# arthur-e/MOD16

Measured on AMD Instinct MI355X. Metric: pixels/sec, fused Penman-Monteith ET forward run (day+night), 43200x21600 global grid, higher is better.
Workload: dtype f64

## Files before the change

### mod16_amd/csrc/capi/internal.hpp

```cpp
#pragma once
#include <hip/hip_runtime.h>

#include <algorithm>
#include <cmath>
#include <cstdio>
#include <cstdlib>
#include <cstring>
#include <limits>
#include <mutex>
#include <new>
#include <string>
#include <thread>
#include <vector>

#include "../../../include/mod16_hip.h"
#include "own.hpp"
#include "../mod16_kernels.hpp"
#include "../mod16_stream.hpp"

using namespace mod16;

namespace {
constexpr int kDiagBlocks = 1024;
constexpr int kSlots = 12;
// ... 105 lines not shown
        used += align256(bytes);
        return p;
    }
};

static void derive_lut(const double* lut, double* h64) {
    const double nan = std::numeric_limits<double>::quiet_NaN();
    for (int c = 0; c < kLutCols; ++c) {
        double row[MOD16_LUT_ROWS];
        for (int k = 0; k < MOD16_LUT_ROWS; ++k) row[k] = nan;
        if (c < MOD16_N_CLASSES) {
            const double* p = lut + (size_t)c * MOD16_N_PARAMS;
            for (int k = 0; k < MOD16_N_PARAMS; ++k) row[k] = p[k];
            row[11] = 1.0 / (p[MOD16_TMIN_OPEN] - p[MOD16_TMIN_CLOSE]);
            row[12] = 1.0 / (p[MOD16_VPD_CLOSE] - p[MOD16_VPD_OPEN]);
            row[13] = (p[MOD16_RBL_MAX] - p[MOD16_RBL_MIN]) / (p[MOD16_VPD_CLOSE] - p[MOD16_VPD_OPEN]);
            row[14] = 1.0 / p[MOD16_BETA];
            const double thr = 273.15 + p[MOD16_TMIN_CLOSE];
            float tf = (float)thr;
            if ((double)tf < thr) tf = std::nextafterf(tf, std::numeric_limits<float>::infinity());
            row[15] = (double)tf;
        }
        for (int k = 0; k < MOD16_LUT_ROWS; ++k) h64[k * kLutCols + c] = row[k];
    }
}

template <typename T> static const T* ctx_lut(const mod16_ctx* ctx);
template <> const double* ctx_lut<double>(const mod16_ctx* ctx) { return ctx->lut64.as<double>(); }
template <> const float* ctx_lut<float>(const mod16_ctx* ctx) { return ctx->lut32.as<float>(); }


// ... 485 lines not shown
```

### mod16_amd/csrc/mod16_composite.hpp

```cpp
#pragma once
#include "mod16_kernels.hpp"

namespace mod16 {

constexpr int kCompArrays = 15;
constexpr int kCompHours = 14;
constexpr int kCompMaxDays = 4096;

template <typename T> struct CompArgs {
    const T* arr[kCompArrays];
    int64_t tstride[kCompArrays];
    int every[kCompArrays];
    uint32_t dense;
    const uint8_t* cls;
    const double* lut64;
    const double* tab;
    T* out_et;
    T* out_pet;
    uint16_t* cnt_et;
    uint16_t* cnt_pet;
    int64_t out_pitch, cnt_pitch, n;
    int days, period_days, min_valid, rescale;
    unsigned* status;
};
// ... 36 lines not shown
__device__ __forceinline__ ClassPar<double> comp_params(const double* l) {
    ClassPar<double> p;
    p.tmin_close = l[0 * kLutCols];
    p.tmin_open = l[1 * kLutCols];
    p.vpd_open = l[2 * kLutCols];
    p.vpd_close = l[3 * kLutCols];
    p.gl_sh = l[4 * kLutCols];
    p.gl_wv = l[5 * kLutCols];
    p.g_cut = l[6 * kLutCols];
    p.csl = l[7 * kLutCols];
    p.rbl_min = l[8 * kLutCols];
    p.rbl_max = l[9 * kLutCols];
    p.beta = l[10 * kLutCols];
    p.inv_dtmin = l[11 * kLutCols];
    p.inv_dvpd = l[12 * kLutCols];
    p.rbl_slope = l[13 * kLutCols];
    p.inv_beta = l[14 * kLutCols];
    return p;
}

__device__ __forceinline__ PixelIn<double> comp_pixel(const double (&v)[kCompArrays]) {
    return PixelIn<double>{v[0], v[1], v[2], v[3], v[4], v[5], v[6], v[7], v[8], v[9], v[10], v[11], v[12], v[13]};
}

template <bool PET>
__device__ __forceinline__ void comp_totals(const PixelOut<double>& o, double h, double& et, double& pet) {
#pragma clang fp contract(off)
    et = comp_daily((o.canopy_d + o.soil_d) + o.trans_d, (o.canopy_n + o.soil_n) + o.trans_n, h);
    pet = PET ? comp_daily(o.pet_d, o.pet_n, h) : 0.0;
}

// ... 156 lines not shown
```

### mod16_amd/csrc/mod16_ensemble.hpp

```cpp
#pragma once
#include "mod16_kernels.hpp"

namespace mod16 {

constexpr int kEnsChunk = 16;
constexpr int kEnsTable = MOD16_LUT_ROWS * kLutCols;
constexpr int64_t kEnsMaxMembers = 65536;
constexpr int kEnsOut = 5;

template <typename T> struct EnsArgs {
    const T* drv[14];
    const uint8_t* cls;
    const double* tables;
    const double* tab;
    T* out[kEnsOut];
    int64_t n;
    int members;
    unsigned* status;
    uint32_t dense_drv;
};

struct EnsPeriod {
    double vpd, logrh, fwet, omw, s, slhv, inv_rcorr, g_rr;
    double rf;
// ... 90 lines not shown

struct EnsMember {
    double vpd_open, inv_dvpd, rbl_min, drbl, inv_beta, gl_sh, g_cut, csl_mt, glsh_lai, glwv_lai;
    bool cond;
};
__device__ __forceinline__ EnsMember ens_member(const EnsPixel& px, const double* l) {
#pragma clang fp contract(off)
    EnsMember m;
    const double tmin_close = l[0 * kLutCols];
    m.vpd_open = l[2 * kLutCols];
    m.gl_sh = l[4 * kLutCols];
    const double gl_wv = l[5 * kLutCols];
    m.g_cut = l[6 * kLutCols];
    const double csl = l[7 * kLutCols];
    m.rbl_min = l[8 * kLutCols];
    const double rbl_max = l[9 * kLutCols];
    const double inv_dtmin = l[11 * kLutCols];
    m.inv_dvpd = l[12 * kLutCols];
    m.inv_beta = l[14 * kLutCols];
    m.cond = px.base_cond & (px.t_ann >= (273.15 + tmin_close));
    m.glsh_lai = m.gl_sh * px.lai;
    m.glwv_lai = gl_wv * px.lai;
    m.drbl = rbl_max - m.rbl_min;
    typedef FastMath<double> M;
    m.csl_mt = csl * M::nan_from(M::mul_unit(px.tm - tmin_close, inv_dtmin), px.tm);
    return m;
}

template <bool DAY>
__device__ __forceinline__ double ens_period_eval(const EnsPixel& px, const EnsPeriod& c, const EnsMember& m,
                                                  const double* tb) {
#pragma clang fp contract(off)
    typedef FastMath<double> M;
    const double tiny = 1e-7;
    const double vramp = M::mul_unit(c.vpd - m.vpd_open, m.inv_dvpd);
    double canopy, soil, trans;
    {
        const double g_e = m.glwv_lai * c.fwet;
// ... 437 lines not shown
```

### mod16_amd/csrc/mod16_kernels.hpp

```cpp
#pragma once
#include <stdint.h>
#include <type_traits>
#include "mod16_physics.hpp"

namespace mod16 {

constexpr int kBlock = 256;
constexpr int kLutCols = 16;
constexpr unsigned kStatusClassRange = 1u;
constexpr unsigned kStatusIncomplete = 2u;
constexpr int kSerialField = 3;
__device__ __forceinline__ double launch_marker(unsigned serial) { return (double)((serial & 0xffffu) + 1u); }

template <typename T> struct EtArgs {
    const T* drv[14];
    const T* par[11];
    const uint8_t* cls;
    const T* lut;
    const double* lut64;
    const double* tab;
    T* out[10];
    int64_t n;
    unsigned* status;
    uint32_t dense_drv;
// ... 126 lines not shown
                const C* l = lut + c;
                p.tmin_close = l[0 * kLutCols];
                p.tmin_open = l[1 * kLutCols];
                p.vpd_open = l[2 * kLutCols];
                p.vpd_close = l[3 * kLutCols];
                p.gl_sh = l[4 * kLutCols];
                p.gl_wv = l[5 * kLutCols];
                p.g_cut = l[6 * kLutCols];
                p.csl = l[7 * kLutCols];
                p.rbl_min = l[8 * kLutCols];
                p.rbl_max = l[9 * kLutCols];
                p.beta = l[10 * kLutCols];
                if (FAST) {
                    p.inv_dtmin = l[11 * kLutCols];
                    p.inv_dvpd = l[12 * kLutCols];
                    p.rbl_slope = l[13 * kLutCols];
                    p.inv_beta = l[14 * kLutCols];
                }
            } else {
                p.tmin_close = (C)par(0);
                p.tmin_open = (C)par(1);
                p.vpd_open = (C)par(2);
                p.vpd_close = (C)par(3);
                p.gl_sh = (C)par(4);
                p.gl_wv = (C)par(5);
                p.g_cut = (C)par(6);
                p.csl = (C)par(7);
                p.rbl_min = (C)par(8);
                p.rbl_max = (C)par(9);
                p.beta = (C)par(10);
                if (FAST) p.derive();
// ... 331 lines not shown
```

### mod16_amd/csrc/mod16_math.hpp

```cpp
#pragma once
#ifndef MOD16_EXPERIMENTS
#if defined(MOD16_TRIVIAL_BODY) || defined(MOD16_NO_GUARD) || defined(MOD16_EXPERIMENT_SEED_RCP) || \
    defined(MOD16_PRIO) || defined(MOD16_REPRO_V4) || defined(MOD16_NO_FUSED_FINAL) ||                \
    defined(MOD16_NO_REDO_LAUNCH) || defined(MOD16_KK_M) || defined(MOD16_NO_FMA_KK) ||               \
    defined(MOD16_DYN_RUN) || defined(MOD16_MIXED_NO_CANCEL) || defined(MOD16_MIXED_CANCEL) || defined(MOD16_F64_CAND)
#error "MOD16_* measurement switches need -DMOD16_EXPERIMENTS (they are not part of the product build)"
#endif
#endif
#include <hip/hip_runtime.h>

namespace mod16 {

__device__ __forceinline__ void ignore_signalling_nans() {
    asm volatile("s_setreg_imm32_b32 hwreg(HW_REG_MODE, 9, 1), 0\n\ts_nop 3" ::: "memory");
}

__device__ __forceinline__ double in_vgpr(double k) {
    asm("" : "+v"(k));
    return k;
}

template <typename T> struct ExactMath {
    static __device__ __forceinline__ T exp(T x);
    static __device__ __forceinline__ T pow(T x, T y);
};
template <> __device__ __forceinline__ double ExactMath<double>::exp(double x) { return ::exp(x); }
template <> __device__ __forceinline__ float ExactMath<float>::exp(float x) { return ::expf(x); }
template <> __device__ __forceinline__ double ExactMath<double>::pow(double x, double y) { return ::pow(x, y); }
template <> __device__ __forceinline__ float ExactMath<float>::pow(float x, float y) { return ::powf(x, y); }

template <typename T> struct FastMath;

template <> struct FastMath<double> {
// ... 54 lines not shown
#else
        return rcp(x);
#endif
    }

    static __device__ __forceinline__ T pow_m1p75(T x) {
        T y = __builtin_amdgcn_sqrt(__builtin_amdgcn_rsq(x));
        T y2 = y * y;
        T t = x * (y2 * y2);
        y = y * fma_kk(t, -0.25, 1.25);
        y2 = y * y;
        T y4 = y2 * y2;
        return (y4 * y2) * y;
    }

    static __device__ __forceinline__ T pow_m1p75_rcp(T x, T& rx) {
        T y = __builtin_amdgcn_sqrt(__builtin_amdgcn_rsq(x));
        T y2 = y * y;
        T t = x * (y2 * y2);
        y = y * fma_kk(t, -0.25, 1.25);
        y2 = y * y;
        T y4 = y2 * y2;
        rx = y4;
        return (y4 * y2) * y;
    }

    static constexpr int kTabRaw = 64 + 2 * 128;
    static constexpr int kTabDoubles = kTabRaw + 16;
    static constexpr double kRintShift = 6755399441055744.0;

    static __device__ __forceinline__ T exp_tab(T x, const T* tb) {
        T km = __builtin_fma(x, 92.33248261689366, kRintShift);
        T kf = km - kRintShift;
        T r = __builtin_fma(kf, -0x1.62e42fee00000p-7, x);
        r = __builtin_fma(kf, -0x1.a39ef35793c76p-39, r);
// ... 7 lines not shown
    }

    static __device__ __forceinline__ T exp_tab4(T x, const T* tb) {
        T km = __builtin_fma(x, 92.33248261689366, kRintShift);
        T kf = km - kRintShift;
        T r = __builtin_fma(kf, -0x1.62e42fee00000p-7, x);
        r = __builtin_fma(kf, -0x1.a39ef35793c76p-39, r);
        T p = fma_kk(r, 1.0 / 24.0, 1.0 / 6.0);
        p = __builtin_fma(p, r, 0.5);
        p = __builtin_fma(p, r, 1.0);
        p = __builtin_fma(p, r, 1.0);
        int ki = __double2loint(km);
        return __builtin_amdgcn_ldexp(tb[ki & 63] * p, ki >> 6);
    }

    static __device__ __forceinline__ T exp_tab4s(T x, const T* tb) {
        T km = __builtin_fma(x, 92.33248261689366, kRintShift);
        T kf = km - kRintShift;
        T r = __builtin_fma(kf, -0.010830424696249145, x);
        T p = fma_kk(r, 1.0 / 24.0, 1.0 / 6.0);
        p = __builtin_fma(p, r, 0.5);
        p = __builtin_fma(p, r, 1.0);
        p = __builtin_fma(p, r, 1.0);
        int ki = __double2loint(km);
        return __builtin_amdgcn_ldexp(tb[ki & 63] * p, ki >> 6);
    }

    static __device__ __forceinline__ T exp_tab5s(T x, const T* tb) {
        T km = __builtin_fma(x, 92.33248261689366, kRintShift);
        T kf = km - kRintShift;
        T r = __builtin_fma(kf, -0.010830424696249145, x);
        T p = fma_kk(r, 1.0 / 120.0, 1.0 / 24.0);
        p = __builtin_fma(p, r, 1.0 / 6.0);
        p = __builtin_fma(p, r, 0.5);
        p = __builtin_fma(p, r, 1.0);
        p = __builtin_fma(p, r, 1.0);
        int ki = __double2loint(km);
        return __builtin_amdgcn_ldexp(tb[ki & 63] * p, ki >> 6);
    }

    static __device__ __forceinline__ T exp_tab3(T x, const T* tb) {
        T km = __builtin_fma(x, 92.33248261689366, kRintShift);
        T kf = km - kRintShift;
        T r = __builtin_fma(kf, -0x1.62e42fee00000p-7, x);
        r = __builtin_fma(kf, -0x1.a39ef35793c76p-39, r);
        T p = fma_kk(r, 1.0 / 6.0, 0.5);
        p = __builtin_fma(p, r, 1.0);
// ... 16 lines not shown
    static __device__ __forceinline__ T log_tab(T x, const T* tb) {
        const unsigned hi = (unsigned)__double2hiint(x);
        const int e = (int)(hi >> 20) - 1023;
        const unsigned j = (hi >> 13) & 127u;
        const T m = __hiloint2double((int)((hi & 0x000fffffu) | 0x3ff00000u), __double2loint(x));
        typedef double d2 __attribute__((ext_vector_type(2)));
        const d2 ent = *reinterpret_cast<const d2*>(tb + 64 + 2 * j);
        T r = __builtin_fma(m, ent[0], -1.0);
        T l1p = log1p_poly(r);
        T ed = (T)e;
        T v = __builtin_fma(ed, 0x1.62e42fefa2000p-1, ent[1]);
        v = v + l1p;
        v = __builtin_fma(ed, 7.371002565167799e-13, v);
        return (x == 0.0) ? -__builtin_huge_val() : v;
    }
    static __device__ __forceinline__ T log_tab1(T x, const T* tb) {
        const unsigned hi = (unsigned)__double2hiint(x);
        const int e = (int)(hi >> 20) - 1023;
        const unsigned j = (hi >> 13) & 127u;
        const T m = __hiloint2double((int)((hi & 0x000fffffu) | 0x3ff00000u), __double2loint(x));
        typedef double d2 __attribute__((ext_vector_type(2)));
        const d2 ent = *reinterpret_cast<const d2*>(tb + 64 + 2 * j);
        T r = __builtin_fma(m, ent[0], -1.0);
        T v = __builtin_fma((T)e, 0.6931471805599453, ent[1]) + log1p_poly(r);
        return (x == 0.0) ? -__builtin_huge_val() : v;
    }
    static __host__ __device__ __forceinline__ T log1p_poly(T r) {
#if defined(__HIP_DEVICE_COMPILE__)
        T p = fma_kk(r, 0.2, -0.25);
#else
        T p = __builtin_fma(r, 0.2, -0.25);
#endif
        p = __builtin_fma(p, r, 1.0 / 3.0);
        p = __builtin_fma(p, r, -0.5);
        return __builtin_fma(r * r, p, r);
    }

    static __device__ __forceinline__ T pow01_tab(T x, T y, const T* tb) {
        T yc = vmin_k(y, 1e300);
        T t = vmax_k(yc * log_tab(x, tb), -746.0);
        return exp_tab4(t, tb);
    }
    static __device__ __forceinline__ T pow01_tab1(T x, T y, const T* tb) {
        T yc = vmin_k(y, 1e300);
        T t = vmax_k(yc * log_tab1(x, tb), -746.0);
        return exp_tab4s(t, tb);
    }
};

}
```

### mod16_amd/csrc/mod16_methods.hpp

```cpp
#pragma once
#include "mod16_kernels.hpp"

namespace mod16 {

constexpr int kMethodMaxIn = 13;

template <typename T> struct MethodArgs {
    const T* in[kMethodMaxIn];
    const T* par[11];
    T* out[2];
    int64_t n;
    uint32_t dense_in, present_in, dense_par;
    int method;
    T alpha;
    T tiny;
};

template <typename T>
__global__ void __launch_bounds__(kBlock) method_kernel(const MethodArgs<T> a) {
    const int64_t step = (int64_t)gridDim.x * kBlock;
    for (int64_t i = (int64_t)blockIdx.x * kBlock + threadIdx.x; i < a.n; i += step) {
        auto has = [&](int k) { return (a.present_in >> k) & 1u; };
        auto in = [&](int k) { return ((a.dense_in >> k) & 1u) ? a.in[k][i] : a.in[k][0]; };
        auto par = [&](int k) { return ((a.dense_par >> k) & 1u) ? a.par[k][i] : a.par[k][0]; };
// ... 743 lines not shown
                      d(12), d(13), a.fpar_pct[i], a.lai_x10[i]};
        unsigned c = a.cls[i];
        if (c >= 13u) {
            atomicOr(a.status, kStatusClassRange);
            c = 13u;
        }
        const C* l = lut + c;
        ClassPar<C> p;
        p.tmin_close = l[0 * kLutCols]; p.tmin_open = l[1 * kLutCols];
        p.vpd_open = l[2 * kLutCols]; p.vpd_close = l[3 * kLutCols];
        p.gl_sh = l[4 * kLutCols]; p.gl_wv = l[5 * kLutCols];
        p.g_cut = l[6 * kLutCols]; p.csl = l[7 * kLutCols];
        p.rbl_min = l[8 * kLutCols]; p.rbl_max = l[9 * kLutCols];
        p.beta = l[10 * kLutCols];
        p.inv_dtmin = l[11 * kLutCols]; p.inv_dvpd = l[12 * kLutCols];
        p.rbl_slope = l[13 * kLutCols]; p.inv_beta = l[14 * kLutCols];
        PixelOut<C> o;
        if constexpr (FAST) {
            double dav_d, dav_n;
            const PixelIn<double> x = raw_to_pixel_fast(r, tab, dav_d, dav_n);
            o = et_pixel_fast<double, false, KLit, true>(x, p, tab, dav_d, dav_n);
            if (raw_out_of_domain(r)) o = et_pixel_exact<double, false, true>(raw_to_pixel_exact<double, true>(r), p);
        } else {
            o = et_pixel_exact<T>(raw_to_pixel_exact<T>(r), p);
        }
        C day = (o.canopy_d + o.soil_d) + o.trans_d;
        C night = (o.canopy_n + o.soil_n) + o.trans_n;
        if (a.out[0]) a.out[0][i] = (T)day;
        if (a.out[1]) a.out[1][i] = (T)night;
        if (a.out[2]) {
#pragma clang fp contract(off)
// ... 9 lines not shown
```

### mod16_amd/csrc/mod16_mixed.hpp

```cpp
#pragma once
#include "mod16_physics.hpp"

namespace mod16 {

typedef float f2 __attribute__((ext_vector_type(2)));

__device__ __forceinline__ f2 splat(float x) { return f2{x, x}; }
__device__ __forceinline__ f2 rcp2(f2 x) {
    f2 r = f2{__builtin_amdgcn_rcpf(x.x), __builtin_amdgcn_rcpf(x.y)};
    f2 e = __builtin_elementwise_fma(-x, r, f2{1.f, 1.f});
    return __builtin_elementwise_fma(r, e, r);
}
__device__ __forceinline__ f2 rcp2_plain(f2 x) { return f2{__builtin_amdgcn_rcpf(x.x), __builtin_amdgcn_rcpf(x.y)}; }
__device__ __forceinline__ f2 clamp01(f2 x) {
    return f2{__builtin_amdgcn_fmed3f(x.x, 0.f, 1.f), __builtin_amdgcn_fmed3f(x.y, 0.f, 1.f)};
}
__device__ __forceinline__ f2 exp2_2(f2 x) { return f2{__builtin_amdgcn_exp2f(x.x), __builtin_amdgcn_exp2f(x.y)}; }
__device__ __forceinline__ f2 log2_2(f2 x) { return f2{__builtin_amdgcn_logf(x.x), __builtin_amdgcn_logf(x.y)}; }
__device__ __forceinline__ f2 sel(bool m0, bool m1, f2 a, f2 b) { return f2{m0 ? a.x : b.x, m1 ? a.y : b.y}; }

__device__ __forceinline__ float lds_f32(const float* p) {
    return *(const volatile __attribute__((address_space(3))) float*)p;
}
constexpr int kLutDrbl = 13;
struct ClassPar2 {
    f2 vpd_open, gl_sh, gl_wv, g_cut, rbl_min, inv_dvpd, drbl, inv_beta;
};

struct Shared2 {
    f2 fpar, omf, p_rel, k_p, p_mbar_k, glwv_l, glsh_lai, csl_m;
    bool lai_pos[2], lai_tiny[2];
};

struct Humid2 {
    f2 esat, rh, fwet, omw;
    bool dry[2];
    bool open_w[2];
};

// ... 382 lines not shown
```

### mod16_amd/csrc/mod16_physics.hpp

```cpp
#pragma once
#include "mod16_math.hpp"

namespace mod16 {

template <typename T> struct PixelIn {
    T lw_d, lw_n, sw_d, sw_n, alb, t_d, t_n, t_ann, tmin, vpd_d, vpd_n, pa,
        fpar, lai;
};

template <typename T> struct ClassPar {
    T tmin_close, tmin_open, vpd_open, vpd_close, gl_sh, gl_wv, g_cut, csl,
        rbl_min, rbl_max, beta;
    T inv_dtmin, inv_dvpd, rbl_slope, inv_beta;
    __device__ __forceinline__ void derive() {
        inv_dtmin = T(1) / (tmin_open - tmin_close);
        inv_dvpd = T(1) / (vpd_close - vpd_open);
        rbl_slope = (rbl_max - rbl_min) / (vpd_close - vpd_open);
        inv_beta = T(1) / beta;
    }
};
#define MOD16_LUT_ROWS 16

template <typename T> struct PixelOut {
    T canopy_d, soil_d, trans_d, canopy_n, soil_n, trans_n;
    T pet_d, pet_n;
};
constexpr double kPriestleyTaylorAlpha = 1.26;

template <typename T> struct K {
    static constexpr T sigma4 = T(4 * 5.67e-8);
    static constexpr T cp = T(1013);
    static constexpr T eps = T(0.622);
    static constexpr T tiny = T(1e-7);
    static constexpr T t0 = T(273.15);
};

// ... 434 lines not shown
        tr = num * M::rcp(den);
    }
    const double r0 = (c.vpd <= p.vpd_open) ? p.rbl_min
                      : ((c.vpd >= p.vpd_close) ? p.rbl_max
                         : __builtin_fma(-(p.vpd_close - c.vpd), d.rbl_slope, p.rbl_max));
    const double r_tot = r0 * c.inv_rc;
    const double w = __builtin_fma(r_tot, c.g_rr, 1.0);
    const double num = __builtin_fma(c.s * rad_soil, r_tot, (c.rcfv * px.omf) * w);
    const double q = num * M::rcp(r_tot * __builtin_fma(c.gamma, w, c.s));
    const double yc = __builtin_fmin(c.vpd * d.inv_beta, 1e300);
    const double pw = M::exp_tab4(__builtin_fmax(yc * c.logrh, -746.0), tb);
    const double e_soil = q * __builtin_fma(c.omw, pw, c.fw);
    return (tr + e_can) + e_soil;
}

struct KLit {
    static __device__ __forceinline__ double per_period(double c) { return c; }
    static __device__ __forceinline__ double per_pixel(double c) { return c; }
};
template <int LEVEL> struct KPin {
    static __device__ __forceinline__ double per_period(double c) { return LEVEL >= 1 ? in_vgpr(c) : c; }
    static __device__ __forceinline__ double per_pixel(double c) { return LEVEL >= 2 ? in_vgpr(c) : c; }
};
#ifndef MOD16_F64_CAND
#define MOD16_F64_CAND 2
#endif
template <typename T> struct PixelShared {
    T oma;
    T omf;
    T p_rel;
    T k_p;
    T p_mbar_k;
    T l_wet;
    T glsh_l, glwv_l;
    T glsh_lai;
    T m_tmin;
    T drbl;
    bool lai_pos, lai_tiny;
};

template <typename T, bool DAY, bool PET = false, typename KP = KLit, bool RAW = false>
__device__ __forceinline__ void period_fast(const PixelIn<T>& x, const ClassPar<T>& p,
                                            const PixelShared<T>& sh, const T* tb, T t, T vpd,
                                            T rad_net, T rad_soil, T& canopy, T& soil,
                                            T& trans, T* pet = nullptr, T dav = T(1)) {
#pragma clang fp contract(off)
    typedef FastMath<T> M;
    const T tiny = K<T>::tiny;
    T tc = t - K<T>::t0;
    T d_es = tc + KP::per_period(237.3);
    T ta = tc + KP::per_period(239.0);
    T dd = d_es * ta;
    T r_both, r_av = T(0);
    if constexpr (RAW) {
        T r3 = M::rcp(dd * dav);
        r_both = r3 * dav;
        r_av = r3 * dd;
    } else {
        r_both = M::rcp(dd);
    }
    T r_es = r_both * ta, rta = r_both * d_es;
    T e_es = M::exp_tab5s((KP::per_period(17.27) * tc) * r_es, tb);
    T esat = T(1e3 * 0.6108) * e_es;
    if constexpr (RAW) {
        T delta = (tc * M::fma_kk(tc, 0x1.c28f5c28f5c00p-4, -0x1.a0c49ba5e34b1p+1)) * r_both;
        T q = M::fma_kk(delta, 1.0 / 720.0, 1.0 / 120.0);
        q = __builtin_fma(q, delta, 1.0 / 24.0);
        q = __builtin_fma(q, delta, 1.0 / 6.0);
        q = __builtin_fma(q, delta, 0.5);
        q = __builtin_fma(q, delta, 1.0);
        q = __builtin_fma(q, delta, 1.0);
        T sv = (T(610.7) * e_es) * q;
        vpd = __builtin_fma(-vpd, r_av, sv);
        if constexpr (!DAY) vpd = (vpd < T(0)) ? T(0) : vpd;
    }
    T avp = esat - vpd;
    T resat = M::rcp(esat);
    T rh = avp * resat;
    rh = M::fma_unit(__builtin_fma(-rh, esat, avp), resat, rh);
    rh = __builtin_fma(avp, T(0), rh);
    T rh2 = rh * rh;
    const bool dry = rh < T(0.7);
    T fwet = dry ? T(0) : rh2 * rh2;
    T omw = T(1) - fwet;
    T s = (KP::per_period(17.38 * 239.0) * esat) * (rta * rta);
    T lhv = M::fma_kk(tc, T(-0.002361e6), T(2.501e6));
    T slhv = s * lhv;
    T rt;
    T inv_rcorr = sh.p_rel * M::pow_m1p75_rcp(t, rt);
    T nn = __builtin_fma(-rh, M::fma_kk(tc, T(0.252 * 1013.0), T(-2.0582 * 1013.0)), sh.p_mbar_k);
    T rho_cp = nn * rt;
    T t2 = t * t;
    T g_rr = (K<T>::sigma4 * (t2 * t2)) * M::rcp(nn);
    T rcfv = rho_cp * vpd;
#if MOD16_F64_CAND >= 2
    T vramp = M::mul_unit(vpd - p.vpd_open, p.inv_dvpd);
#endif

    {
        T fw = fwet;
        T g_e = sh.glwv_l * fw;
        T g_a = __builtin_fma(sh.glsh_l, fw, g_rr);
        T numer = fw * __builtin_fma(rcfv * x.fpar, g_a, s * (x.fpar * rad_net));
        T den = __builtin_fma(slhv, g_e, sh.k_p * g_a);
        T evap = (numer * g_e) * M::rcp_quotient(den);
        canopy = ((numer < T(0)) | dry | sh.lai_tiny) ? T(0) : evap;
    }
    {
#if MOD16_F64_CAND >= 2
        T r0 = __builtin_fma(vramp, sh.drbl, p.rbl_min);
#else
        T r0 = __builtin_fma(-(p.vpd_close - vpd), p.rbl_slope, p.rbl_max);
        r0 = (vpd >= p.vpd_close) ? p.rbl_max : r0;
        r0 = (vpd <= p.vpd_open) ? p.rbl_min : r0;
#endif
        T r_tot = r0 * inv_rcorr;
        T w = __builtin_fma(r_tot, g_rr, T(1));
        T num = __builtin_fma((s * rad_soil), r_tot, (rcfv * sh.omf) * w);
        T den = r_tot * __builtin_fma(sh.k_p, w, slhv);
        T q = num * M::rcp_quotient(den);
        T pw = M::pow01_tab1(rh, vpd * p.inv_beta, tb);
        T e = q * __builtin_fma(omw, pw, fwet);
        soil = (q < T(0)) ? T(0) : e;
        if (PET) {
            T pot_soil = (q < T(0)) ? T(0) : __builtin_fma(q, fwet, q * omw);
            T pot_tr = (T(kPriestleyTaylorAlpha) * (s * (x.fpar * rad_net)) * omw) *
                       M::rcp(__builtin_fma(s, lhv, sh.k_p));
            *pet = (canopy + pot_soil) + pot_tr;
        }
    }
    {
        T g_s = T(0);
        if (DAY) {
#if MOD16_F64_CAND >= 2
            T m_vpd = T(1) - vramp;
#else
// ... 9 lines not shown
        T s1 = __builtin_fma(sh.glsh_lai, omw, gsc);
        bool open = sh.lai_pos & (omw > T(0));
        bool shut = !open | (p1 <= tiny * s1);
        T g_d = p.gl_sh + g_rr;
        T rad_c = x.fpar * rad_net;
        rad_c = (rad_c < T(0)) ? T(0) : rad_c;
        T num = (omw * __builtin_fma(rcfv * x.fpar, g_d, s * rad_c)) * p1;
        T den = __builtin_fma(slhv, p1, sh.k_p * __builtin_fma(g_d, s1, p1));
        T tr = num * M::rcp_quotient(den);
        trans = shut ? T(0) : tr;
    }
}

template <typename T, bool PET = false, typename KP = KLit, bool RAW = false>
__device__ __forceinline__ PixelOut<T> et_pixel_fast(const PixelIn<T>& x, const ClassPar<T>& p,
                                                     const T* tb, T dav_d = T(1), T dav_n = T(1)) {
#pragma clang fp contract(off)
    PixelOut<T> o;
#ifdef MOD16_TRIVIAL_BODY
    o.canopy_d = x.lw_d + x.sw_d + x.alb + x.t_d + x.t_ann + x.vpd_d + x.pa;
    o.soil_d = p.beta; o.trans_d = x.fpar;
    o.canopy_n = x.lw_n + x.sw_n + x.t_n + x.tmin + x.vpd_n + x.lai;
    o.soil_n = p.csl; o.trans_n = p.gl_sh;
    return o;
#endif
    PixelShared<T> sh;
    sh.oma = T(1) - x.alb;
    sh.omf = T(1) - x.fpar;
    T a_d = __builtin_fma(x.sw_d, sh.oma, x.lw_d);
    T a_n = x.lw_n;
    const T k473 = KP::per_pixel(4.73), k2087 = KP::per_pixel(-20.87), k039 = KP::per_pixel(0.39);
// ... 14 lines not shown
#if MOD16_F64_CAND >= 1
    sh.l_wet = x.lai;
    sh.lai_tiny = x.lai <= K<T>::tiny;
    sh.lai_pos = x.lai > T(0);
    sh.glsh_lai = p.gl_sh * x.lai;
    sh.glsh_l = sh.glsh_lai;
    sh.glwv_l = p.gl_wv * x.lai;
#else
    sh.l_wet = (x.lai == T(0)) ? K<T>::tiny : x.lai;
    sh.lai_tiny = sh.l_wet <= K<T>::tiny;
    sh.lai_pos = x.lai > T(0);
    sh.glsh_l = p.gl_sh * sh.l_wet;
    sh.glwv_l = p.gl_wv * sh.l_wet;
    sh.glsh_lai = p.gl_sh * x.lai;
#endif
    sh.drbl = p.rbl_max - p.rbl_min;
    T tm = x.tmin - K<T>::t0;
    typedef FastMath<T> M;
    sh.m_tmin = M::nan_from(M::mul_unit(tm - p.tmin_close, p.inv_dtmin), tm);
    period_fast<T, true, PET, KP, RAW>(x, p, sh, tb, x.t_d, x.vpd_d, a_d, rs_d, o.canopy_d, o.soil_d, o.trans_d,
                                       &o.pet_d, dav_d);
    T rn_n = __builtin_fma(x.sw_n, sh.oma, x.lw_n);
    period_fast<T, false, PET, KP, RAW>(x, p, sh, tb, x.t_n, x.vpd_n, rn_n, rs_n, o.canopy_n, o.soil_n, o.trans_n,
                                        &o.pet_n, dav_n);
    return o;
}

__device__ __forceinline__ double max_abs(double a, double b) {
    double d;
    asm("v_max_f64 %0, |%1|, |%2|" : "=v"(d) : "v"(a), "v"(b));
    return d;
}
__device__ __forceinline__ double max_abs_signed(double a, double b) {
    double d;
    asm("v_max_f64 %0, |%1|, %2" : "=v"(d) : "v"(a), "v"(b));
    return d;
}
constexpr double kGuardHuge = 1e50;
constexpr double kGuardTmin = 36.0;
// ... 116 lines not shown
```

### mod16_amd/csrc/mod16_stream.hpp

```cpp
#pragma once
#include "mod16_kernels.hpp"
#include "mod16_mixed.hpp"

namespace mod16 {

typedef const __attribute__((address_space(1))) void* gptr_t;
typedef __attribute__((address_space(3))) void* lptr_t;
constexpr int kDmaNt = 2;
#ifndef MOD16_DYN_RUN
#define MOD16_DYN_RUN 8
#endif
constexpr int kDynRun = MOD16_DYN_RUN;
constexpr int kPinLevel = 1;

enum StreamMode {
    kStreamPet = 0, kStreamSep8, kStreamSep6, kStreamRaw, kStreamRawTotal, kStreamRawTotalHours,
    kStreamTotals,
    kStreamTotalsMixed, kStreamPetMixed, kStreamSep8Mixed, kStreamSep6Mixed,
    kStreamRawMixed, kStreamRawTotalMixed, kStreamRawTotalHoursMixed
};
constexpr bool stream_is_mixed(int mode) { return mode >= kStreamTotalsMixed; }

template <int MODE> struct StreamSpec;
template <> struct StreamSpec<kStreamTotals> { static constexpr int NW = 14, NB = 1, NOUT = 2; };
// ... 151 lines not shown
    p.tmin_close = l[0 * kLutCols];
    p.tmin_open = l[1 * kLutCols];
    p.vpd_open = l[2 * kLutCols];
    p.vpd_close = l[3 * kLutCols];
    p.gl_sh = l[4 * kLutCols];
    p.gl_wv = l[5 * kLutCols];
    p.g_cut = l[6 * kLutCols];
    p.csl = l[7 * kLutCols];
    p.rbl_min = l[8 * kLutCols];
    p.rbl_max = l[9 * kLutCols];
    p.beta = l[10 * kLutCols];
    PixelOut<double> o;
    if (cancel) {
        p.inv_dtmin = l[11 * kLutCols];
        p.inv_dvpd = l[12 * kLutCols];
        p.rbl_slope = l[13 * kLutCols];
        p.inv_beta = l[14 * kLutCols];
        o = et_pixel_fast<double, kPet>(x, p, tb);
    } else {
        if constexpr (!LISTED) o = et_pixel_exact<double, kPet, true>(x, p);
    }
    const double day = (o.canopy_d + o.soil_d) + o.trans_d;
    const double night = (o.canopy_n + o.soil_n) + o.trans_n;
    auto put = [&](int k, double val) { a.out[k][oo] = (T)val; };
    if constexpr (kSep6) {
        put(0, o.canopy_d); put(1, o.soil_d); put(2, o.trans_d);
        put(3, o.canopy_n); put(4, o.soil_n); put(5, o.trans_n);
    } else {
        put(0, day);
        put(1, night);
    }
// ... 205 lines not shown
            else
                __builtin_amdgcn_global_load_lds((gptr_t)((p.b[k] + first) + (lb >> 2)),
                                                 (lptr_t)(uintptr_t)(wl + NW * 1024 + k * 256), 4, 0, kDmaNt);
        }
    };
    {
        Ptrs p;
        load_ptrs(p);
        const Offs of = offs_of(cbase + run);
        out_first = of.o;
        if (lane < lanes) issue(of, p);
    }
    for (int i = threadIdx.x; i < MOD16_LUT_ROWS * kLutCols; i += kBlock) {
        const double x = a.lut64[i];
        lut[i] = x;
        if constexpr (stream_is_mixed(MODE))
            lut32[i] = i / kLutCols == kLutDrbl ? (float)(a.lut64[9 * kLutCols + i % kLutCols] - a.lut64[8 * kLutCols + i % kLutCols])
                                                : (float)x;
    }
    for (int i = threadIdx.x; i < kTab; i += kBlock) tab[i] = a.tab[i];
    __syncthreads();
    asm volatile("s_waitcnt vmcnt(0)" ::: "memory");
    const GuardConsts gc = RAW ? raw_guard_consts() : guard_consts();
#pragma nounroll
    for (; cbase + run < npiece; ) {
        Ptrs ptrs;
#ifdef MOD16_PRIO
        __builtin_amdgcn_s_setprio(MOD16_PRIO);
#endif
        load_ptrs(ptrs);
        asm volatile("s_waitcnt vmcnt(%0)" ::"n"(NOUT) : "memory");
        if (__builtin_expect(run == claim_run, 0)) {
            asm volatile("" : "+v"(ticket));
            const unsigned lo = __builtin_amdgcn_readfirstlane((unsigned)ticket);
            const unsigned hi = __builtin_amdgcn_readfirstlane((unsigned)(ticket >> 32));
            const unsigned past = ((unsigned)npiece >> rs) + 1u;
            const unsigned tk = (hi != 0u || lo > past) ? past : lo;
            next_base = (int)(((unsigned)nwaves + tk) << rs);
// ... 164 lines not shown
                const double* l = lut + c;
                ClassPar<double> p;
                p.tmin_close = l[0 * kLutCols];
                p.tmin_open = l[1 * kLutCols];
                p.vpd_open = l[2 * kLutCols];
                p.vpd_close = l[3 * kLutCols];
                p.gl_sh = l[4 * kLutCols];
                p.gl_wv = l[5 * kLutCols];
                p.g_cut = l[6 * kLutCols];
                p.csl = l[7 * kLutCols];
                p.rbl_min = l[8 * kLutCols];
                p.rbl_max = l[9 * kLutCols];
                p.beta = l[10 * kLutCols];
                p.inv_dtmin = l[11 * kLutCols];
                p.inv_dvpd = l[12 * kLutCols];
                p.rbl_slope = l[13 * kLutCols];
                p.inv_beta = l[14 * kLutCols];
                typedef typename std::conditional<MODE == kStreamTotals && std::is_same<T, double>::value, KPin<kPinLevel>, KLit>::type KP;
                PixelOut<double> o = et_pixel_fast<double, MODE == kStreamPet, KP, RAW>(x, p, tab, dav_d, dav_n);
                const double day = (o.canopy_d + o.soil_d) + o.trans_d;
                const double night = (o.canopy_n + o.soil_n) + o.trans_n;
                if constexpr (MODE == kStreamSep6) {
                    res[0][j] = (T)o.canopy_d; res[1][j] = (T)o.soil_d; res[2][j] = (T)o.trans_d;
                    res[3][j] = (T)o.canopy_n; res[4][j] = (T)o.soil_n; res[5][j] = (T)o.trans_n;
                } else {
                    res[0][j] = (T)day;
                    res[1][j] = (T)night;
                }
                if constexpr (MODE == kStreamPet) {
                    res[2][j] = (T)o.pet_d;
                    res[3][j] = (T)o.pet_n;
                }
                if constexpr (MODE == kStreamSep8) {
                    res[2][j] = (T)o.canopy_d; res[3][j] = (T)o.soil_d; res[4][j] = (T)o.trans_d;
// ... 264 lines not shown
```

Before: 49.12 billion.

## Hoist polynomial constants into loop-invariant VGPRs and precompute drbl in LUT

Adds a KHeld policy that materializes the f64 polynomial and physics constants once per kernel into VGPRs via volatile asm, before the streaming loop. Each per-pixel FMA then uses a register operand instead of rematerializing a 64-bit literal with extra instructions. It also replaces the unused rbl_slope LUT row with a precomputed drbl (rbl_max - rbl_min), removing a per-pixel subtraction and the special-cased f32 LUT fill. The cost is higher VGPR pressure, which could reduce occupancy.

```diff
diff --git a/mod16_amd/csrc/capi/internal.hpp b/mod16_amd/csrc/capi/internal.hpp
--- a/mod16_amd/csrc/capi/internal.hpp
+++ b/mod16_amd/csrc/capi/internal.hpp
@@ -143,7 +143,7 @@
             for (int k = 0; k < MOD16_N_PARAMS; ++k) row[k] = p[k];
             row[11] = 1.0 / (p[MOD16_TMIN_OPEN] - p[MOD16_TMIN_CLOSE]);
             row[12] = 1.0 / (p[MOD16_VPD_CLOSE] - p[MOD16_VPD_OPEN]);
-            row[13] = (p[MOD16_RBL_MAX] - p[MOD16_RBL_MIN]) / (p[MOD16_VPD_CLOSE] - p[MOD16_VPD_OPEN]);
+            row[13] = p[MOD16_RBL_MAX] - p[MOD16_RBL_MIN];
             row[14] = 1.0 / p[MOD16_BETA];
             const double thr = 273.15 + p[MOD16_TMIN_CLOSE];
             float tf = (float)thr;
diff --git a/mod16_amd/csrc/mod16_composite.hpp b/mod16_amd/csrc/mod16_composite.hpp
--- a/mod16_amd/csrc/mod16_composite.hpp
+++ b/mod16_amd/csrc/mod16_composite.hpp
@@ -74,7 +74,7 @@
     p.beta = l[10 * kLutCols];
     p.inv_dtmin = l[11 * kLutCols];
     p.inv_dvpd = l[12 * kLutCols];
-    p.rbl_slope = l[13 * kLutCols];
+    p.drbl = l[kLutDrbl * kLutCols];
     p.inv_beta = l[14 * kLutCols];
     return p;
 }
diff --git a/mod16_amd/csrc/mod16_ensemble.hpp b/mod16_amd/csrc/mod16_ensemble.hpp
--- a/mod16_amd/csrc/mod16_ensemble.hpp
+++ b/mod16_amd/csrc/mod16_ensemble.hpp
@@ -128,14 +128,13 @@
     m.g_cut = l[6 * kLutCols];
     const double csl = l[7 * kLutCols];
     m.rbl_min = l[8 * kLutCols];
-    const double rbl_max = l[9 * kLutCols];
     const double inv_dtmin = l[11 * kLutCols];
     m.inv_dvpd = l[12 * kLutCols];
     m.inv_beta = l[14 * kLutCols];
     m.cond = px.base_cond & (px.t_ann >= (273.15 + tmin_close));
     m.glsh_lai = m.gl_sh * px.lai;
     m.glwv_lai = gl_wv * px.lai;
-    m.drbl = rbl_max - m.rbl_min;
+    m.drbl = l[kLutDrbl * kLutCols];
     typedef FastMath<double> M;
     m.csl_mt = csl * M::nan_from(M::mul_unit(px.tm - tmin_close, inv_dtmin), px.tm);
     return m;
diff --git a/mod16_amd/csrc/mod16_kernels.hpp b/mod16_amd/csrc/mod16_kernels.hpp
--- a/mod16_amd/csrc/mod16_kernels.hpp
+++ b/mod16_amd/csrc/mod16_kernels.hpp
@@ -164,7 +164,7 @@
                 if (FAST) {
                     p.inv_dtmin = l[11 * kLutCols];
                     p.inv_dvpd = l[12 * kLutCols];
-                    p.rbl_slope = l[13 * kLutCols];
+                    p.drbl = l[kLutDrbl * kLutCols];
                     p.inv_beta = l[14 * kLutCols];
                 }
             } else {
diff --git a/mod16_amd/csrc/mod16_math.hpp b/mod16_amd/csrc/mod16_math.hpp
--- a/mod16_amd/csrc/mod16_math.hpp
+++ b/mod16_amd/csrc/mod16_math.hpp
@@ -17,6 +17,11 @@
 
 __device__ __forceinline__ double in_vgpr(double k) {
     asm("" : "+v"(k));
+    return k;
+}
+
+__device__ __forceinline__ double held_in_vgpr(double k) {
+    asm volatile("" : "+v"(k));
     return k;
 }
 
@@ -101,11 +106,11 @@
         return (y4 * y2) * y;
     }
 
-    static __device__ __forceinline__ T pow_m1p75_rcp(T x, T& rx) {
+    static __device__ __forceinline__ T pow_m1p75_rcp(T x, T& rx, T kk_m = -0.25, T kk_c = 1.25) {
         T y = __builtin_amdgcn_sqrt(__builtin_amdgcn_rsq(x));
         T y2 = y * y;
         T t = x * (y2 * y2);
-        y = y * fma_kk(t, -0.25, 1.25);
+        y = y * fma_kk(t, kk_m, kk_c);
         y2 = y * y;
         T y4 = y2 * y2;
         rx = y4;
@@ -143,23 +148,23 @@
         return __builtin_amdgcn_ldexp(tb[ki & 63] * p, ki >> 6);
     }
 
-    static __device__ __forceinline__ T exp_tab4s(T x, const T* tb) {
+    static __device__ __forceinline__ T exp_tab4s(T x, const T* tb, T kk_m = 1.0 / 24.0, T kk_c = 1.0 / 6.0) {
         T km = __builtin_fma(x, 92.33248261689366, kRintShift);
         T kf = km - kRintShift;
         T r = __builtin_fma(kf, -0.010830424696249145, x);
-        T p = fma_kk(r, 1.0 / 24.0, 1.0 / 6.0);
-        p = __builtin_fma(p, r, 0.5);
-        p = __builtin_fma(p, r, 1.0);
-        p = __builtin_fma(p, r, 1.0);
-        int ki = __double2loint(km);
-        return __builtin_amdgcn_ldexp(tb[ki & 63] * p, ki >> 6);
-    }
-
-    static __device__ __forceinline__ T exp_tab5s(T x, const T* tb) {
+        T p = fma_kk(r, kk_m, kk_c);
+        p = __builtin_fma(p, r, 0.5);
+        p = __builtin_fma(p, r, 1.0);
+        p = __builtin_fma(p, r, 1.0);
+        int ki = __double2loint(km);
+        return __builtin_amdgcn_ldexp(tb[ki & 63] * p, ki >> 6);
+    }
+
+    static __device__ __forceinline__ T exp_tab5s(T x, const T* tb, T kk_m = 1.0 / 120.0, T kk_c = 1.0 / 24.0) {
         T km = __builtin_fma(x, 92.33248261689366, kRintShift);
         T kf = km - kRintShift;
         T r = __builtin_fma(kf, -0.010830424696249145, x);
-        T p = fma_kk(r, 1.0 / 120.0, 1.0 / 24.0);
+        T p = fma_kk(r, kk_m, kk_c);
         p = __builtin_fma(p, r, 1.0 / 6.0);
         p = __builtin_fma(p, r, 0.5);
         p = __builtin_fma(p, r, 1.0);
@@ -206,7 +211,7 @@
         v = __builtin_fma(ed, 7.371002565167799e-13, v);
         return (x == 0.0) ? -__builtin_huge_val() : v;
     }
-    static __device__ __forceinline__ T log_tab1(T x, const T* tb) {
+    static __device__ __forceinline__ T log_tab1(T x, const T* tb, T kk_m = 0.2, T kk_c = -0.25) {
         const unsigned hi = (unsigned)__double2hiint(x);
         const int e = (int)(hi >> 20) - 1023;
         const unsigned j = (hi >> 13) & 127u;
@@ -214,14 +219,14 @@
         typedef double d2 __attribute__((ext_vector_type(2)));
         const d2 ent = *reinterpret_cast<const d2*>(tb + 64 + 2 * j);
         T r = __builtin_fma(m, ent[0], -1.0);
-        T v = __builtin_fma((T)e, 0.6931471805599453, ent[1]) + log1p_poly(r);
+        T v = __builtin_fma((T)e, 0.6931471805599453, ent[1]) + log1p_poly(r, kk_m, kk_c);
         return (x == 0.0) ? -__builtin_huge_val() : v;
     }
-    static __host__ __device__ __forceinline__ T log1p_poly(T r) {
+    static __host__ __device__ __forceinline__ T log1p_poly(T r, T kk_m = 0.2, T kk_c = -0.25) {
 #if defined(__HIP_DEVICE_COMPILE__)
-        T p = fma_kk(r, 0.2, -0.25);
+        T p = fma_kk(r, kk_m, kk_c);
 #else
-        T p = __builtin_fma(r, 0.2, -0.25);
+        T p = __builtin_fma(r, kk_m, kk_c);
 #endif
         p = __builtin_fma(p, r, 1.0 / 3.0);
         p = __builtin_fma(p, r, -0.5);
@@ -233,10 +238,11 @@
         T t = vmax_k(yc * log_tab(x, tb), -746.0);
         return exp_tab4(t, tb);
     }
-    static __device__ __forceinline__ T pow01_tab1(T x, T y, const T* tb) {
+    static __device__ __forceinline__ T pow01_tab1(T x, T y, const T* tb, T log_m = 0.2, T log_c = -0.25,
+                                                   T exp_m = 1.0 / 24.0, T exp_c = 1.0 / 6.0) {
         T yc = vmin_k(y, 1e300);
-        T t = vmax_k(yc * log_tab1(x, tb), -746.0);
-        return exp_tab4s(t, tb);
+        T t = vmax_k(yc * log_tab1(x, tb, log_m, log_c), -746.0);
+        return exp_tab4s(t, tb, exp_m, exp_c);
     }
 };
 
diff --git a/mod16_amd/csrc/mod16_methods.hpp b/mod16_amd/csrc/mod16_methods.hpp
--- a/mod16_amd/csrc/mod16_methods.hpp
+++ b/mod16_amd/csrc/mod16_methods.hpp
@@ -781,7 +781,7 @@
         p.rbl_min = l[8 * kLutCols]; p.rbl_max = l[9 * kLutCols];
         p.beta = l[10 * kLutCols];
         p.inv_dtmin = l[11 * kLutCols]; p.inv_dvpd = l[12 * kLutCols];
-        p.rbl_slope = l[13 * kLutCols]; p.inv_beta = l[14 * kLutCols];
+        p.drbl = l[kLutDrbl * kLutCols]; p.inv_beta = l[14 * kLutCols];
         PixelOut<C> o;
         if constexpr (FAST) {
             double dav_d, dav_n;
diff --git a/mod16_amd/csrc/mod16_mixed.hpp b/mod16_amd/csrc/mod16_mixed.hpp
--- a/mod16_amd/csrc/mod16_mixed.hpp
+++ b/mod16_amd/csrc/mod16_mixed.hpp
@@ -22,7 +22,6 @@
 __device__ __forceinline__ float lds_f32(const float* p) {
     return *(const volatile __attribute__((address_space(3))) float*)p;
 }
-constexpr int kLutDrbl = 13;
 struct ClassPar2 {
     f2 vpd_open, gl_sh, gl_wv, g_cut, rbl_min, inv_dvpd, drbl, inv_beta;
 };
diff --git a/mod16_amd/csrc/mod16_physics.hpp b/mod16_amd/csrc/mod16_physics.hpp
--- a/mod16_amd/csrc/mod16_physics.hpp
+++ b/mod16_amd/csrc/mod16_physics.hpp
@@ -11,15 +11,16 @@
 template <typename T> struct ClassPar {
     T tmin_close, tmin_open, vpd_open, vpd_close, gl_sh, gl_wv, g_cut, csl,
         rbl_min, rbl_max, beta;
-    T inv_dtmin, inv_dvpd, rbl_slope, inv_beta;
+    T inv_dtmin, inv_dvpd, drbl, inv_beta;
     __device__ __forceinline__ void derive() {
         inv_dtmin = T(1) / (tmin_open - tmin_close);
         inv_dvpd = T(1) / (vpd_close - vpd_open);
-        rbl_slope = (rbl_max - rbl_min) / (vpd_close - vpd_open);
+        drbl = rbl_max - rbl_min;
         inv_beta = T(1) / beta;
     }
 };
 #define MOD16_LUT_ROWS 16
+constexpr int kLutDrbl = 13;
 
 template <typename T> struct PixelOut {
     T canopy_d, soil_d, trans_d, canopy_n, soil_n, trans_n;
@@ -484,13 +485,29 @@
     return (tr + e_can) + e_soil;
 }
 
-struct KLit {
+#define MOD16_FAST_KK(X)                                                                            \
+    X(exp5_m, 1.0 / 120.0) X(k24, 1.0 / 24.0) X(k6, 1.0 / 6.0) X(log_m, 0.2) X(kq, -0.25) X(pw_c, 1.25) \
+    X(lhv_m, -0.002361e6) X(lhv_c, 2.501e6) X(nn_m, 0.252 * 1013.0) X(nn_c, -2.0582 * 1013.0)
+struct KKLit {
+#define MOD16_X(name, value) __device__ __forceinline__ double name() const { return value; }
+    MOD16_FAST_KK(MOD16_X)
+#undef MOD16_X
+};
+struct KLit : KKLit {
     static __device__ __forceinline__ double per_period(double c) { return c; }
     static __device__ __forceinline__ double per_pixel(double c) { return c; }
 };
-template <int LEVEL> struct KPin {
+template <int LEVEL> struct KPin : KKLit {
     static __device__ __forceinline__ double per_period(double c) { return LEVEL >= 1 ? in_vgpr(c) : c; }
     static __device__ __forceinline__ double per_pixel(double c) { return LEVEL >= 2 ? in_vgpr(c) : c; }
+};
+template <int LEVEL> struct KHeld {
+    static __device__ __forceinline__ double per_period(double c) { return KPin<LEVEL>::per_period(c); }
+    static __device__ __forceinline__ double per_pixel(double c) { return KPin<LEVEL>::per_pixel(c); }
+#define MOD16_X(name, value) double name##_ = held_in_vgpr(value); \
+    __device__ __forceinline__ double name() const { return name##_; }
+    MOD16_FAST_KK(MOD16_X)
+#undef MOD16_X
 };
 #ifndef MOD16_F64_CAND
 #define MOD16_F64_CAND 2
@@ -505,7 +522,6 @@
     T glsh_l, glwv_l;
     T glsh_lai;
     T m_tmin;
-    T drbl;
     bool lai_pos, lai_tiny;
 };
 
@@ -513,7 +529,7 @@
 __device__ __forceinline__ void period_fast(const PixelIn<T>& x, const ClassPar<T>& p,
                                             const PixelShared<T>& sh, const T* tb, T t, T vpd,
                                             T rad_net, T rad_soil, T& canopy, T& soil,
-                                            T& trans, T* pet = nullptr, T dav = T(1)) {
+                                            T& trans, T* pet = nullptr, T dav = T(1), const KP& kp = KP()) {
 #pragma clang fp contract(off)
     typedef FastMath<T> M;
     const T tiny = K<T>::tiny;
@@ -530,7 +546,7 @@
         r_both = M::rcp(dd);
     }
     T r_es = r_both * ta, rta = r_both * d_es;
-    T e_es = M::exp_tab5s((KP::per_period(17.27) * tc) * r_es, tb);
+    T e_es = M::exp_tab5s((KP::per_period(17.27) * tc) * r_es, tb, kp.exp5_m(), kp.k24());
     T esat = T(1e3 * 0.6108) * e_es;
     if constexpr (RAW) {
         T delta = (tc * M::fma_kk(tc, 0x1.c28f5c28f5c00p-4, -0x1.a0c49ba5e34b1p+1)) * r_both;
@@ -554,11 +570,11 @@
     T fwet = dry ? T(0) : rh2 * rh2;
     T omw = T(1) - fwet;
     T s = (KP::per_period(17.38 * 239.0) * esat) * (rta * rta);
-    T lhv = M::fma_kk(tc, T(-0.002361e6), T(2.501e6));
+    T lhv = M::fma_kk(tc, kp.lhv_m(), kp.lhv_c());
     T slhv = s * lhv;
     T rt;
-    T inv_rcorr = sh.p_rel * M::pow_m1p75_rcp(t, rt);
-    T nn = __builtin_fma(-rh, M::fma_kk(tc, T(0.252 * 1013.0), T(-2.0582 * 1013.0)), sh.p_mbar_k);
+    T inv_rcorr = sh.p_rel * M::pow_m1p75_rcp(t, rt, kp.kq(), kp.pw_c());
+    T nn = __builtin_fma(-rh, M::fma_kk(tc, kp.nn_m(), kp.nn_c()), sh.p_mbar_k);
     T rho_cp = nn * rt;
     T t2 = t * t;
     T g_rr = (K<T>::sigma4 * (t2 * t2)) * M::rcp(nn);
@@ -578,9 +594,9 @@
     }
     {
 #if MOD16_F64_CAND >= 2
-        T r0 = __builtin_fma(vramp, sh.drbl, p.rbl_min);
+        T r0 = __builtin_fma(vramp, p.drbl, p.rbl_min);
 #else
-        T r0 = __builtin_fma(-(p.vpd_close - vpd), p.rbl_slope, p.rbl_max);
+        T r0 = __builtin_fma(-(p.vpd_close - vpd), p.drbl * p.inv_dvpd, p.rbl_max);
         r0 = (vpd >= p.vpd_close) ? p.rbl_max : r0;
         r0 = (vpd <= p.vpd_open) ? p.rbl_min : r0;
 #endif
@@ -589,7 +605,7 @@
         T num = __builtin_fma((s * rad_soil), r_tot, (rcfv * sh.omf) * w);
         T den = r_tot * __builtin_fma(sh.k_p, w, slhv);
         T q = num * M::rcp_quotient(den);
-        T pw = M::pow01_tab1(rh, vpd * p.inv_beta, tb);
+        T pw = M::pow01_tab1(rh, vpd * p.inv_beta, tb, kp.log_m(), kp.kq(), kp.k24(), kp.k6());
         T e = q * __builtin_fma(omw, pw, fwet);
         soil = (q < T(0)) ? T(0) : e;
         if (PET) {
@@ -629,7 +645,7 @@
 
 template <typename T, bool PET = false, typename KP = KLit, bool RAW = false>
 __device__ __forceinline__ PixelOut<T> et_pixel_fast(const PixelIn<T>& x, const ClassPar<T>& p,
-                                                     const T* tb, T dav_d = T(1), T dav_n = T(1)) {
+                                                     const T* tb, T dav_d = T(1), T dav_n = T(1), const KP& kp = KP()) {
 #pragma clang fp contract(off)
     PixelOut<T> o;
 #ifdef MOD16_TRIVIAL_BODY
@@ -674,15 +690,14 @@
     sh.glwv_l = p.gl_wv * sh.l_wet;
     sh.glsh_lai = p.gl_sh * x.lai;
 #endif
-    sh.drbl = p.rbl_max - p.rbl_min;
     T tm = x.tmin - K<T>::t0;
     typedef FastMath<T> M;
     sh.m_tmin = M::nan_from(M::mul_unit(tm - p.tmin_close, p.inv_dtmin), tm);
     period_fast<T, true, PET, KP, RAW>(x, p, sh, tb, x.t_d, x.vpd_d, a_d, rs_d, o.canopy_d, o.soil_d, o.trans_d,
-                                       &o.pet_d, dav_d);
+                                       &o.pet_d, dav_d, kp);
     T rn_n = __builtin_fma(x.sw_n, sh.oma, x.lw_n);
     period_fast<T, false, PET, KP, RAW>(x, p, sh, tb, x.t_n, x.vpd_n, rn_n, rs_n, o.canopy_n, o.soil_n, o.trans_n,
-                                        &o.pet_n, dav_n);
+                                        &o.pet_n, dav_n, kp);
     return o;
 }
 
diff --git a/mod16_amd/csrc/mod16_stream.hpp b/mod16_amd/csrc/mod16_stream.hpp
--- a/mod16_amd/csrc/mod16_stream.hpp
+++ b/mod16_amd/csrc/mod16_stream.hpp
@@ -189,7 +189,7 @@
     if (cancel) {
         p.inv_dtmin = l[11 * kLutCols];
         p.inv_dvpd = l[12 * kLutCols];
-        p.rbl_slope = l[13 * kLutCols];
+        p.drbl = l[kLutDrbl * kLutCols];
         p.inv_beta = l[14 * kLutCols];
         o = et_pixel_fast<double, kPet>(x, p, tb);
     } else {
@@ -425,14 +425,14 @@
     for (int i = threadIdx.x; i < MOD16_LUT_ROWS * kLutCols; i += kBlock) {
         const double x = a.lut64[i];
         lut[i] = x;
-        if constexpr (stream_is_mixed(MODE))
-            lut32[i] = i / kLutCols == kLutDrbl ? (float)(a.lut64[9 * kLutCols + i % kLutCols] - a.lut64[8 * kLutCols + i % kLutCols])
-                                                : (float)x;
+        if constexpr (stream_is_mixed(MODE)) lut32[i] = (float)x;
     }
     for (int i = threadIdx.x; i < kTab; i += kBlock) tab[i] = a.tab[i];
     __syncthreads();
     asm volatile("s_waitcnt vmcnt(0)" ::: "memory");
     const GuardConsts gc = RAW ? raw_guard_consts() : guard_consts();
+    typedef typename std::conditional<MODE == kStreamTotals && std::is_same<T, double>::value, KHeld<kPinLevel>, KLit>::type KP;
+    const KP kp;
 #pragma nounroll
     for (; cbase + run < npiece; ) {
         Ptrs ptrs;
@@ -627,10 +627,9 @@
                 p.beta = l[10 * kLutCols];
                 p.inv_dtmin = l[11 * kLutCols];
                 p.inv_dvpd = l[12 * kLutCols];
-                p.rbl_slope = l[13 * kLutCols];
+                p.drbl = l[kLutDrbl * kLutCols];
                 p.inv_beta = l[14 * kLutCols];
-                typedef typename std::conditional<MODE == kStreamTotals && std::is_same<T, double>::value, KPin<kPinLevel>, KLit>::type KP;
-                PixelOut<double> o = et_pixel_fast<double, MODE == kStreamPet, KP, RAW>(x, p, tab, dav_d, dav_n);
+                PixelOut<double> o = et_pixel_fast<double, MODE == kStreamPet, KP, RAW>(x, p, tab, dav_d, dav_n, kp);
                 const double day = (o.canopy_d + o.soil_d) + o.trans_d;
                 const double night = (o.canopy_n + o.soil_n) + o.trans_n;
                 if constexpr (MODE == kStreamSep6) {
```

Result: no change. 49.38 billion, median of 6 (+0.5%).
